# JaronTu/Multimodal_MVD_Seg

Measured on AMD Instinct MI355X. Metric: train-step samples/sec on 4-modality 128^3 patches (PlainConvUNet 3d_fullres, fp32), higher is better.
Workload: dtype f32; 1 GPU; BASELINE configs[1]: PlainConvUNet 3d_fullres 6 stages 31.2M params, 4x128x128x128 patch, 5 classes, fp32, DC+CE deep supervision, SGD-Nesterov+clip; per_gpu_batch=2, global_batch=2, parallelism=dp1, step_launch=one hipGraph replay per step (captured after 3 eager steps)

## Files before the change

### include/mvdseg_hip.h

```cpp
#ifndef MVDSEG_HIP_H
#define MVDSEG_HIP_H
#include <stddef.h>
#include <stdint.h>

#ifdef __cplusplus
extern "C" {
#endif

#define MVD_VERSION 100
#define MVD_MAX_TAPS 27

int mvd_version(void);
const char *mvd_last_error(void);
int mvd_has_mfma(void);
int mvd_set_conv_engine(int mode);
int mvd_set_wino_min_items(long n);

int mvd_pack_weight(const float *w, float *wf, float *wb, int K, int C, int T, int transposed, void *stream);

size_t mvd_conv_fwd_workspace_bytes(int N, long out_voxels, int K);
int mvd_conv3d_fwd(const float *x1, int C1, const float *x2, int C2, const float *wf, const float *bias, float *y,
                   int N, int D, int H, int W, int K, const int ksize[3], const int stride[3], void *ws,
                   size_t ws_bytes, void *stream);
int mvd_conv3d_dgrad(const float *dy, const float *wb, float *dx1, int C1, float *dx2, int C2, int N, int D, int H,
// ... 42 lines not shown
#define MVD_WG_MFMA 5
#define MVD_WG_WGRAD16 6
#define MVD_WG_WGRAD16Z 7
#define MVD_WG_WGRAD16ZS 8
#define MVD_WG_SCALAR 9
#define MVD_WG_PLAN_LEN 34
#define MVD_WGR_F4 1
#define MVD_WGR_F16 2
#define MVD_WGR_WINO 3
#define MVD_WGR_WINO2 4
#define MVD_WGR_WINO3 5
#define MVD_WGR_D 6
#define MVD_WGB_NONE 0
#define MVD_WGB_COLSUM 1
#define MVD_WGB_GENERIC 2
#define MVD_WGB_CONVT 3
#define MVD_WGB_SMALLC 4
#define MVD_WGB_WINO3 5
#define MVD_WGB_WINO2W12 6
#define MVD_WGB_SLOT28 7
#define MVD_WGB_ZMARCH 8
int mvd_conv_wgrad_plan(int transposed, int is_bf16, int N, int D, int H, int W, int C1, int C2, int K, const int ksize[3],
                        const int stride[3], size_t ws_bytes, int want_bias, int prologue, long *plan);
int mvd_conv_wgrad_last_kernel(void);
size_t mvd_conv3d_wgrad_workspace_bytes(int C, int K, int T, int N, int Do, int Ho, int Wo);
int mvd_conv3d_wgrad(const float *x1, int C1, const float *x2, int C2, const float *dy, float *dw, float *dbias,
                     int N, int D, int H, int W, int K, const int ksize[3], const int stride[3], void *ws,
                     size_t ws_bytes, void *stream);

int mvd_convT3d_fwd(const float *x, const float *wf, const float *bias, float *y, int N, int D, int H, int W, int C,
                    int K, const int stride[3], void *ws, size_t ws_bytes, void *stream);
int mvd_convT3d_dgrad(const float *dy, const float *wb, float *dx, int N, int D, int H, int W, int C, int K,
                      const int stride[3], void *ws, size_t ws_bytes, void *stream);
size_t mvd_convT3d_wgrad_workspace_bytes(int C, int K, int T, int N, int D, int H, int W);
int mvd_convT3d_wgrad(const float *x, const float *dy, float *dw, float *dbias, int N, int D, int H, int W, int C,
                      int K, const int stride[3], void *ws, size_t ws_bytes, void *stream);

int mvd_pack_weight_bf16(const float *w, uint16_t *wf, uint16_t *wb, int K, int C, int T, int transposed, void *stream);
int mvd_pack_weights_bf16_batch(int n, const float *const *w, uint16_t *const *wf, uint16_t *const *wb, const int *K,
                                const int *C, const int *T, const int *transposed, void *stream);
int mvd_pack_weights_bf16_batch_pad(int n, const float *const *w, uint16_t *const *wf, uint16_t *const *wb, const int *K,
                                    const int *C, const int *T, const int *transposed, const int *Csrc, void *stream);
int mvd_conv3d_fwd_bf16(const uint16_t *x1, int C1, const uint16_t *x2, int C2, const uint16_t *wf, const float *bias,
                        uint16_t *y, int N, int D, int H, int W, int K, const int ksize[3], const int stride[3],
                        void *ws, size_t ws_bytes, void *stream);
int mvd_conv3d_dgrad_bf16(const uint16_t *dy, const uint16_t *wb, uint16_t *dx1, int C1, uint16_t *dx2, int C2, int N,
                          int D, int H, int W, int K, const int ksize[3], const int stride[3], void *ws, size_t ws_bytes,
                          void *stream);
int mvd_convT3d_fwd_bf16(const uint16_t *x, const uint16_t *wf, const float *bias, uint16_t *y, int N, int D, int H, int W,
                         int C, int K, const int stride[3], void *ws, size_t ws_bytes, void *stream);
int mvd_convT3d_dgrad_bf16(const uint16_t *dy, const uint16_t *wb, uint16_t *dx, int N, int D, int H, int W, int C, int K,
                           const int stride[3], void *ws, size_t ws_bytes, void *stream);
int mvd_conv3d_wgrad_bf16(const uint16_t *x1, int C1, const uint16_t *x2, int C2, const uint16_t *dy, float *dw,
                          float *dbias, int N, int D, int H, int W, int K, const int ksize[3], const int stride[3],
                          void *ws, size_t ws_bytes, void *stream);
int mvd_convT3d_wgrad_bf16(const uint16_t *x, const uint16_t *dy, float *dw, float *dbias, int N, int D, int H, int W,
                           int C, int K, const int stride[3], void *ws, size_t ws_bytes, void *stream);
int mvd_conv3d_fwd_bf16_stats_tiles(int N, int D, int H, int W, int C1, int C2, int K, const int ksize[3],
                                    const int stride[3]);
int mvd_conv3d_dgrad_acc_ok(int is_bf16, int N, int D, int H, int W, int C1, int K, const int ksize[3], const int stride[3]);
int mvd_conv3d_dgrad_acc(const float *dy, const float *wb, float *dx1, int C1, int N, int D, int H, int W, int K,
                         const int ksize[3], const int stride[3], void *stream);
int mvd_conv3d_dgrad_bf16_acc(const uint16_t *dy, const uint16_t *wb, uint16_t *dx1, int C1, int N, int D, int H, int W, int K,
                              const int ksize[3], const int stride[3], void *ws, size_t ws_bytes, void *stream);
int mvd_set_bf16_zmarch_kernel(int which);
int mvd_set_bf16_wgrad_kernel(int which);
// ... 387 lines not shown
```

### multimodal_mvd_seg_amd/_lib.py

```python
import ctypes
import os
from ctypes import c_double, c_float, c_int, c_long, c_size_t, c_uint64, c_void_p

_HERE = os.path.dirname(os.path.abspath(__file__))
LIB_PATH = os.path.join(_HERE, "libmvdseg_hip.so")

_P = c_void_p
_I3 = ctypes.c_int * 3

CONV_DIRECT, CONV_WINO2, CONV_WINO3, CONV_WINO2P = 0, 1, 2, 3

SIGNATURES = {
    "mvd_version": (c_int, []),
    "mvd_last_error": (ctypes.c_char_p, []),
    "mvd_has_mfma": (c_int, []),
    "mvd_set_conv_engine": (c_int, [c_int]),
    "mvd_set_wino_min_items": (c_int, [c_long]),
    "mvd_pack_weight": (c_int, [_P, _P, _P, c_int, c_int, c_int, c_int, _P]),
    "mvd_conv_fwd_workspace_bytes": (c_size_t, [c_int, c_long, c_int]),
    "mvd_conv3d_fwd": (c_int, [_P, c_int, _P, c_int, _P, _P, _P, c_int, c_int, c_int, c_int, c_int, _I3, _I3, _P,
                               c_size_t, _P]),
    "mvd_conv3d_dgrad": (c_int, [_P, _P, _P, c_int, _P, c_int, c_int, c_int, c_int, c_int, c_int, _I3, _I3, _P,
                                 c_size_t, _P]),
    "mvd_conv3d_wgrad_workspace_bytes": (c_size_t, [c_int, c_int, c_int, c_int, c_int, c_int, c_int]),
    "mvd_conv3d_wgrad": (c_int, [_P, c_int, _P, c_int, _P, _P, _P, c_int, c_int, c_int, c_int, c_int, _I3, _I3, _P,
                                 c_size_t, _P]),
    "mvd_convT3d_fwd": (c_int, [_P, _P, _P, _P, c_int, c_int, c_int, c_int, c_int, c_int, _I3, _P, c_size_t, _P]),
    "mvd_convT3d_dgrad": (c_int, [_P, _P, _P, c_int, c_int, c_int, c_int, c_int, c_int, _I3, _P, c_size_t, _P]),
    "mvd_convT3d_wgrad_workspace_bytes": (c_size_t, [c_int, c_int, c_int, c_int, c_int, c_int, c_int]),
    "mvd_convT3d_wgrad": (c_int, [_P, _P, _P, _P, c_int, c_int, c_int, c_int, c_int, c_int, _I3, _P, c_size_t, _P]),
    "mvd_conv3d_route": (c_int, [c_int, c_int, c_int, c_int, c_int, c_int, c_int, _I3, _I3]),
    "mvd_conv3d_fwd_routed": (c_int, [_P, c_int, _P, c_int, _P, _P, c_int, _P, _P, _P, c_long, _P, c_int, c_int, c_int, c_int,
                                      c_int, _I3, _I3, _P, c_size_t, _P]),
    "mvd_conv3d_dgrad_routed": (c_int, [_P, _P, _P, c_int, _P, c_int, _P, c_int, c_int, c_int, c_int, c_int, c_int, _I3, _I3, _P,
                                        c_size_t, _P]),
    "mvd_conv_wino_applicable": (c_int, [c_int, c_int, c_int, c_int, c_int, c_int, c_int, _I3, _I3]),
    "mvd_wino_mode": (c_int, []),
    "mvd_wino_weight_elems": (c_size_t, [c_int, c_int]),
    "mvd_pack_weight_wino": (c_int, [_P, _P, _P, c_int, c_int, _P]),
    "mvd_conv3d_fwd_wino": (c_int, [_P, c_int, _P, c_int, _P, _P, _P, _P, c_int, c_int, c_int, c_int, c_int, _I3, _I3, _P,
                                    c_size_t, _P]),
    "mvd_conv_stats_tiles": (c_size_t, [c_int, c_int, c_int]),
    "mvd_conv3d_fwd_stats_tiles": (c_long, [c_int, c_int, c_int, c_int, c_int, c_int, c_int, _I3, _I3]),
    "mvd_set_wino3_min_items": (c_int, [c_long]),
    "mvd_conv_wino3_applicable": (c_int, [c_int, c_int, c_int, c_int, c_int, c_int, c_int, _I3, _I3]),
    "mvd_wino3_weight_elems": (c_size_t, [c_int, c_int]),
    "mvd_pack_weight_wino3": (c_int, [_P, _P, _P, c_int, c_int, _P]),
    "mvd_pack_weights_batch3": (c_int, [c_int] + [_P] * 11 + [_P]),
    "mvd_set_wino2p_min_items": (c_int, [c_long]),
    "mvd_conv_wino2p_applicable": (c_int, [c_int, c_int, c_int, c_int, c_int, c_int, c_int, _I3, _I3]),
    "mvd_wino2p_weight_elems": (c_size_t, [c_int, c_int]),
    "mvd_pack_weight_wino2p": (c_int, [_P, _P, _P, c_int, c_int, _P]),
    "mvd_set_wgrad_wino3_min_items": (c_int, [c_long]),
    "mvd_conv_wgrad_wino3_applicable": (c_int, [c_int, c_int, c_int, c_int, c_int, c_int, c_int, _I3, _I3]),
    "mvd_wgrad_wino3_launches": (c_long, []),
    "mvd_set_wgrad_bias_fold": (c_int, [c_int]),
    "mvd_conv_wgrad_plan": (c_int, [c_int, c_int, c_int, c_int, c_int, c_int, c_int, c_int, c_int, _I3, _I3, c_size_t, c_int,
                                    c_int, _P]),
    "mvd_conv_wgrad_last_kernel": (c_int, []),
    "mvd_conv3d_wgrad_bf16": (c_int, [_P, c_int, _P, c_int, _P, _P, _P, c_int, c_int, c_int, c_int, c_int, _I3, _I3, _P,
                                      c_size_t, _P]),
# ... 257 lines not shown
```

### multimodal_mvd_seg_amd/csrc/conv.hip

```cpp
#include "common.h"
#include "conv_geom.h"

namespace mvd {

static int g_engine_mode = 0;
#define g_wino_off (wino_mode() == 0)
static const int g_transp_off = getenv("MVD_TRANSP") ? (atoi(getenv("MVD_TRANSP")) == 0) : 0;
static long g_wino_min_items = getenv("MVD_WINO_MIN") ? atol(getenv("MVD_WINO_MIN")) : 256;
static const long kWino3MinItemsDefault = 128;
static long g_wino3_min_items = getenv("MVD_WINO3_MIN") ? atol(getenv("MVD_WINO3_MIN")) : kWino3MinItemsDefault;
static const long kWino2pMinItemsDefault = 256;
static long g_wino2p_min_items = getenv("MVD_WINO2P_MIN") ? atol(getenv("MVD_WINO2P_MIN")) : kWino2pMinItemsDefault;

struct ConvPass {
    int N, D, H, W, R1, R2, P1, P2;
    const int *ks, *st;
};
static ConvPass fwd_pass(int N, int D, int H, int W, int C1, int C2, int K, const int ks[3], const int st[3]) {
    return {N, D, H, W, C1, C2, K, 0, ks, st};
}
static ConvPass dgrad_pass(int N, int D, int H, int W, int C1, int C2, int K, const int ks[3], const int st[3]) {
    return {N, D, H, W, K, 0, C1, C2, ks, st};
}
static bool wino_pass_ok(const ConvPass &p, int kd) {
    if (g_engine_mode != 0 || g_wino_off || !p.ks || !p.st) return false;
    if (p.ks[0] != kd || p.ks[1] != 3 || p.ks[2] != 3 || p.st[0] != 1 || p.st[1] != 1 || p.st[2] != 1) return false;
    if (p.N <= 0 || p.D <= 0 || p.H <= 0 || p.W <= 0 || p.R1 <= 0 || p.R2 < 0 || p.P1 <= 0 || p.P2 < 0) return false;
    return !(p.R1 % 32 || p.R2 % 32 || p.P1 % 32 || p.P2 % 32);
}
static long wino2_items(int N, int D, int H, int W, int K) { return (long)N * ((D + 3) / 4) * ((H + 3) / 4) * ((W + 7) / 8) * (K / 32); }
static bool wino2_takes(const ConvPass &p) {
    return wino_pass_ok(p, 3) && wino2_items(p.N, p.D, p.H, p.W, p.P1 + p.P2) >= g_wino_min_items;
}
static long wino3_items(int D, int H, int W, int K) { return (long)((D + 3) / 4) * ((H + 7) / 8) * ((W + 7) / 8) * (K / 32); }
static bool wino3_takes(const ConvPass &p) {
    return wino3_enabled() && wino2_takes(p) && wino3_items(p.D, p.H, p.W, p.P1 + p.P2) >= g_wino3_min_items;
}
static bool wino2p_takes(const ConvPass &p) {
    if (!wino_pass_ok(p, 1)) return false;
    const int cmax = p.R1 + p.R2 > p.P1 + p.P2 ? p.R1 + p.R2 : p.P1 + p.P2;
// ... 582 lines not shown
    if (want_bias && !in_kernel_bias) p.bias_src = WGB_COLSUM;
    const long out[MVD_WG_PLAN_LEN] = {p.kernel, p.reduce, p.bias_src, p.TPW, p.NA, p.NB, p.SH, p.TRI, p.TD, p.TH, p.TW,
                                       p.ntd, p.nth, p.ntw, p.ntiles, p.nsplit, p.partials, p.ncb, p.nkb, p.bias_rows,
                                       (long)p.needed_ws, (long)p.ws_bytes, p.wino_mode, p.wino3_on, p.wino3_min_items,
                                       p.bias_fold, p.bf16_kernel, p.engine_mode, p.env_big16, p.env_tri16, p.env_db,
                                       p.env_16z, p.env_16zs, p.env_reduce_g16};
    for (int i = 0; i < MVD_WG_PLAN_LEN; i++) plan[i] = out[i];
    return 0;
}

int mvd_set_wgrad_bias_fold(int on) {
    set_wgrad_bias_fold(on);
    return 0;
}

int mvd_conv3d_wgrad(const float *x1, int C1, const float *x2, int C2, const float *dy, float *dw, float *dbias, int N,
                     int D, int H, int W, int K, const int ksize[3], const int stride[3], void *ws, size_t ws_bytes,
                     void *stream) {
    MVD_REQUIRE(x1 && dy && dw && ws && C1 > 0 && C2 >= 0 && (C2 == 0 || x2), "conv3d_wgrad: null pointer / bad channels");
    MVD_REQUIRE(N > 0 && D > 0 && H > 0 && W > 0 && K > 0, "conv3d_wgrad: bad shape");
    if (check_ks(ksize, stride, "conv3d_wgrad")) return 2;
    WgradGeom g;
    conv_wgrad_geom(g, N, D, H, W, C1, C2, K, ksize, stride);
    MVD_REQUIRE(ws_bytes >= mvd_conv3d_wgrad_workspace_bytes(C1 + C2, K, g.T, N, g.Do, g.Ho, g.Wo),
                "conv3d_wgrad: workspace too small");
    hipStream_t s = as_stream(stream);
    int dbias_done = 0;
    int r = run_wgrad(g, x1, x2, dy, dw, ws, ws_bytes, s, dbias, &dbias_done);
    if (r) return r;
    if (dbias && !dbias_done) return colsum(dy, dbias, (long)N * g.Do * g.Ho * g.Wo, K, ws, s);
    return 0;
}

int mvd_convT3d_fwd(const float *x, const float *wf, const float *bias, float *y, int N, int D, int H, int W, int C, int K,
                    const int stride[3], void *ws, size_t ws_bytes, void *stream) {
    MVD_REQUIRE(x && wf && y && N > 0 && D > 0 && H > 0 && W > 0 && C > 0 && K > 0, "convT3d_fwd: bad arguments");
    for (int a = 0; a < 3; a++) MVD_REQUIRE(stride[a] == 1 || stride[a] == 2, "convT3d_fwd: stride must be 1 or 2");
    if (g_engine_mode == 0 && !g_transp_off) {
        int r = convT_fwd_direct(x, wf, bias, y, N, D, H, W, C, K, stride, as_stream(stream));
        if (r >= 0) return r;
    }
    for (int pd = 0; pd < stride[0]; pd++)
        for (int ph = 0; ph < stride[1]; ph++)
            for (int pw = 0; pw < stride[2]; pw++) {
                const int p[3] = {pd, ph, pw};
                FwdGeom g;
                convT_fwd_class_geom(g, N, D, H, W, C, K, stride, p);
                int r = run_fwd(g, x, nullptr, wf, bias, y, nullptr, ws, ws_bytes, as_stream(stream));
                if (r) return r;
            }
    return 0;
}

int mvd_convT3d_dgrad(const float *dy, const float *wb, float *dx, int N, int D, int H, int W, int C, int K,
                      const int stride[3], void *ws, size_t ws_bytes, void *stream) {
    MVD_REQUIRE(dy && wb && dx && N > 0 && D > 0 && H > 0 && W > 0 && C > 0 && K > 0, "convT3d_dgrad: bad arguments");
    for (int a = 0; a < 3; a++) MVD_REQUIRE(stride[a] == 1 || stride[a] == 2, "convT3d_dgrad: stride must be 1 or 2");
    if (g_engine_mode == 0 && !g_transp_off) {
        int r = convT_dgrad_direct(dy, wb, dx, N, D, H, W, C, K, stride, as_stream(stream));
        if (r >= 0) return r;
    }
    FwdGeom g;
    convT_dgrad_geom(g, N, D, H, W, C, K, stride);
    return run_fwd(g, dy, nullptr, wb, nullptr, dx, nullptr, ws, ws_bytes, as_stream(stream));
}

size_t mvd_convT3d_wgrad_workspace_bytes(int C, int K, int T, int N, int D, int H, int W) {
    WgradGeom g;
    memset(&g, 0, sizeof(g));
    g.N = N; g.Do = D; g.Ho = H; g.Wo = W; g.C1 = C; g.K = K; g.ntaps = g.T = T;
    size_t a = max_sz(wgrad_scalar_ws(g), wgrad_mfma_ws(g));
    return max_sz(a, colsum_ws((long)N * D * H * W * T, K));
}

int mvd_convT3d_wgrad(const float *x, const float *dy, float *dw, float *dbias, int N, int D, int H, int W, int C, int K,
                      const int stride[3], void *ws, size_t ws_bytes, void *stream) {
    MVD_REQUIRE(x && dy && dw && ws && N > 0 && D > 0 && H > 0 && W > 0 && C > 0 && K > 0, "convT3d_wgrad: bad arguments");
    for (int a = 0; a < 3; a++) MVD_REQUIRE(stride[a] == 1 || stride[a] == 2, "convT3d_wgrad: stride must be 1 or 2");
    WgradGeom g;
    convT_wgrad_geom(g, N, D, H, W, C, K, stride);
    MVD_REQUIRE(ws_bytes >= mvd_convT3d_wgrad_workspace_bytes(C, K, g.T, N, D, H, W), "convT3d_wgrad: workspace too small");
    hipStream_t s = as_stream(stream);
    int dbias_done = 0;
    int r = run_wgrad(g, x, nullptr, dy, dw, ws, ws_bytes, s, dbias, &dbias_done);
    if (r) return r;
    if (dbias && !dbias_done) return colsum(dy, dbias, (long)N * g.Db * g.Hb * g.Wb, K, ws, s);
    return 0;
}

int mvd_pack_weight_bf16(const float *w, uint16_t *wf, uint16_t *wb, int K, int C, int T, int transposed, void *stream) {
    MVD_REQUIRE(w && (wf || wb) && K > 0 && C > 0 && T > 0 && T <= MVD_MAX_TAPS, "pack_weight_bf16: bad arguments");
    MVD_REQUIRE(!wf || C % 32 == 0, "pack_weight_bf16: wf needs C %% 32 == 0");
    MVD_REQUIRE(!wb || K % 32 == 0, "pack_weight_bf16: wb needs K %% 32 == 0");
    return pack_weight16(w, wf, wb, K, C, T, transposed, as_stream(stream));
// ... 257 lines not shown
```

### multimodal_mvd_seg_amd/csrc/conv_geom.h

```cpp
#pragma once
#include <hip/hip_runtime.h>
#include <stdint.h>
#include <string.h>

namespace mvd {

__host__ __device__ inline int wl_ck(int C) {
    return (C % 32 == 0) ? 32 : ((C % 8 == 0) ? 8 : ((C % 4 == 0) ? 4 : 0));
}
__host__ __device__ inline size_t widx(int CK, int T, int C, int K, int t, int c, int k) {
    if (CK == 0) return ((size_t)t * C + c) * K + k;
    const int hh = CK / 2;
    const int cc = c / CK, r = c % CK;
    return ((((size_t)cc * T + t) * 2 + r / hh) * K + k) * hh + (r % hh);
}

struct FwdGeom {
    int N;
    int T;
    int Di, Hi, Wi;
    int Do, Ho, Wo;
    int Dy, Hy, Wy;
    int C1, C2, K1, K2;
    int ntaps;
// ... 262 lines not shown

int fwd_wino(const FwdGeom &g, const float *a1, const float *a2, const float *u, const float *bias, float *y1, float *y2,
             hipStream_t s, float *stats = nullptr, int *stats_done = nullptr);
int pack_weight_wino(const float *w, float *uf, float *ub, int K, int C, hipStream_t s);
int fwd_wino3(const FwdGeom &g, const float *a1, const float *a2, const float *u, const float *bias, float *y1, float *y2,
              hipStream_t s, float *stats = nullptr, int *stats_done = nullptr);
int pack_weight_wino3(const float *w, float *uf, float *ub, int K, int C, hipStream_t s);
int wino3_enabled();
int fwd_wino2p(const FwdGeom &g, const float *a1, const float *a2, const float *u, const float *bias, float *y1, float *y2,
               hipStream_t s);
int pack_weight_wino2p(const float *w, float *uf, float *ub, int K, int C, hipStream_t s);
long wino2p_items(int N, int D, int H, int W, int K);
int dgrad32s(int N, int D, int H, int W, int C, int K, int Do, int Ho, int Wo, const float *dy, const float *wb, float *dx,
             hipStream_t s, int accumulate = 0);
int dgrad16s(int N, int D, int H, int W, int C, int K, int Do, int Ho, int Wo, const unsigned short *dy, const unsigned short *wb,
             unsigned short *dx, hipStream_t s, int accumulate = 0);
int launch_fwd16ys(const FwdGeom &g, const unsigned short *a1, const unsigned short *a2, const unsigned short *w, const float *bias,
                   unsigned short *y1, unsigned short *y2, hipStream_t s, int ncu);
bool wgrad16z_prologue_ok(const WgradGeom &g);
void wgrad16z_enable(int on);
int pack_weights_batch(int n, const float *const *w, float *const *wf, float *const *wb, float *const *uf, float *const *ub,
                       const int *K, const int *C, const int *T, const int *transposed, hipStream_t s,
                       float *const *vf = nullptr, float *const *vb = nullptr);
int wino_mode();
bool wgrad_wino3_selected(const WgradGeom &g);
size_t wgrad_wino3_ws(int nsplit, int C, int K);
int wgrad_wino3_enabled();
void set_wgrad_wino3_min_items(long n);
void set_wgrad_bias_fold(int on);
long wgrad_wino3_launches();
int dbias_reduce(const float *pbias, float *dbias, int K, int nrows, hipStream_t s);
size_t wino_weight_elems(int C, int K);

int convT_fwd_direct(const float *x, const float *wf, const float *bias, float *y, int N, int D, int H, int W, int C, int K,
                     const int st[3], hipStream_t s);
int convT_dgrad_direct(const float *dy, const float *wb, float *dx, int N, int D, int H, int W, int C, int K,
                       const int st[3], hipStream_t s);

int convT_fwd_direct16(const unsigned short *x, const unsigned short *wf, const float *bias, unsigned short *y, int N, int D,
                       int H, int W, int C, int K, const int st[3], hipStream_t s);
int convT_dgrad_direct16(const unsigned short *dy, const unsigned short *wb, unsigned short *dx, int N, int D, int H, int W,
                         int C, int K, const int st[3], hipStream_t s);

struct Fwd16Fuse {
    float *tile_stats = nullptr;
    int *ntiles = nullptr;
    const float *in_scale = nullptr, *in_shift = nullptr;
    float slope = 0.01f;
};
int fwd_bf16(const FwdGeom &g, const unsigned short *a1, const unsigned short *a2, const unsigned short *w,
             const float *bias, unsigned short *y1, unsigned short *y2, void *ws, size_t ws_bytes, hipStream_t s,
             const Fwd16Fuse *fuse = nullptr);
int fwd16y_enabled();
void fwd16y_enable(int on);
int launch_fwd16y(const FwdGeom &g, const unsigned short *a1, const unsigned short *a2, const unsigned short *w,
                  const float *bias, unsigned short *y1, unsigned short *y2, hipStream_t s, const Fwd16Fuse *fuse, int ncu,
                  int *stats_tiles_only);
int fwd_bf16_stats_tiles(const FwdGeom &g);
int fwd_bf16_prologue_ok(const FwdGeom &g);
int pack_weight16(const float *w, unsigned short *wf, unsigned short *wb, int K, int C, int T, int transposed,
                  hipStream_t s);
int pack_weights16_batch(int n, const float *const *w, unsigned short *const *wf, unsigned short *const *wb, const int *K,
                         const int *C, const int *T, const int *transposed, const int *Csrc, hipStream_t s);

}
```

### multimodal_mvd_seg_amd/csrc/conv_transp.hip

```cpp
#include <algorithm>
#include <stdlib.h>
#include "common.h"
#include "conv_geom.h"

namespace mvd {

typedef float f32x16 __attribute__((ext_vector_type(16)));

struct TranspGeom {
    int N, D, H, W, C, K;
    int s[3], T;
    long NV;
};

__device__ inline long out_base(const TranspGeom &g, unsigned v) {
    const unsigned t1 = v / (unsigned)g.W, w = v - t1 * (unsigned)g.W;
    const unsigned t2 = t1 / (unsigned)g.H, h = t1 - t2 * (unsigned)g.H;
    return (((long)t2 * g.s[0]) * (g.H * g.s[1]) + (long)h * g.s[1]) * (g.W * g.s[2]) + (long)w * g.s[2];
}

__global__ __launch_bounds__(256, 4) void k_convT_fwd(const TranspGeom g, const float *__restrict__ x,
                                                      const float *__restrict__ wf, const float *__restrict__ bias,
                                                      float *__restrict__ y) {
    const int lane = threadIdx.x & 63;
// ... 211 lines not shown
                for (int e = 0; e < 4; e++) a[u ^ 1][e] = *reinterpret_cast<const float4 *>(pa + e * 4);
#pragma unroll
                for (int q = 0; q < NT; q++)
#pragma unroll
                    for (int e = 0; e < 4; e++)
                        b[u ^ 1][q][e] = (cb0 + q < ncb) ? *reinterpret_cast<const float4 *>(pb + (size_t)q * 512 + e * 4)
                                                         : make_float4(0.f, 0.f, 0.f, 0.f);
#pragma unroll
                for (int e = 0; e < 4; e++) {
#pragma unroll
                    for (int q = 0; q < NT; q++) acc[q] = __builtin_amdgcn_mfma_f32_32x32x2f32(a[u][e].x, b[u][q][e].x, acc[q], 0, 0, 0);
#pragma unroll
                    for (int q = 0; q < NT; q++) acc[q] = __builtin_amdgcn_mfma_f32_32x32x2f32(a[u][e].y, b[u][q][e].y, acc[q], 0, 0, 0);
#pragma unroll
                    for (int q = 0; q < NT; q++) acc[q] = __builtin_amdgcn_mfma_f32_32x32x2f32(a[u][e].z, b[u][q][e].z, acc[q], 0, 0, 0);
#pragma unroll
                    for (int q = 0; q < NT; q++) acc[q] = __builtin_amdgcn_mfma_f32_32x32x2f32(a[u][e].w, b[u][q][e].w, acc[q], 0, 0, 0);
                }
            }
        }
    }
#pragma unroll
    for (int q = 0; q < NT; q++)
        if (cb0 + q < ncb) {
            const int c = (cb0 + q) * 32 + i;
#pragma unroll
            for (int r = 0; r < 16; r++) {
                const int row = (r & 3) + 8 * (r >> 2) + 4 * h;
                if (vb + row < g.NV) dx[(size_t)(vb + row) * g.C + c] = acc[q][r];
            }
        }
}

__global__ __launch_bounds__(256, 2) void k_convT_dgrad_p(const TranspGeom g, const float *__restrict__ dy,
                                                         const float *__restrict__ wb, float *__restrict__ dx, int ngrp) {
    const int lane = threadIdx.x & 63;
    const int wave = __builtin_amdgcn_readfirstlane(threadIdx.x >> 6);
    const int i = lane & 31, h = lane >> 5;
    const int ncb = g.C >> 5;
    const int cb = wave % ncb;
    const int gsub = wave / ncb, gper = 4 / ncb;
    const int Hy = g.H * g.s[1], Wy = g.W * g.s[2];
    const float *wl = wb + (((size_t)h * g.C + cb * 32 + i) << 4);
    const size_t wtap = (size_t)2 * g.C * 16;
    float4 wr[8][4];
    int poff[8];
#pragma unroll
    for (int p = 0; p < 8; p++) {
#pragma unroll
        for (int e = 0; e < 4; e++) wr[p][e] = *reinterpret_cast<const float4 *>(wl + (size_t)p * wtap + e * 4);
        const int pw = p % g.s[2], ph = (p / g.s[2]) % g.s[1], pd = p / (g.s[2] * g.s[1]);
        poff[p] = (pd * Hy + ph) * Wy + pw;
    }
    const int c = cb * 32 + i;
    const int gstride = (int)gridDim.x * gper;
    int grp = (int)blockIdx.x * gper + gsub;
    if (grp >= ngrp) return;
    auto row_ptr = [&](int gq) {
        const long vv = (long)gq * 32 + i;
        const long ob = out_base(g, (unsigned)(vv < g.NV ? vv : g.NV - 1));
        return dy + (size_t)ob * g.K + h * 16;
    };
    const float *rp = row_ptr(grp);
    float4 a[2][4];
#pragma unroll
    for (int e = 0; e < 4; e++) a[0][e] = *reinterpret_cast<const float4 *>(rp + (size_t)poff[0] * g.K + e * 4);
    for (; grp < ngrp; grp += gstride) {
        const int gn = grp + gstride < ngrp ? grp + gstride : grp;
        const float *rn = row_ptr(gn);
        f32x16 acc;
#pragma unroll
        for (int r = 0; r < 16; r++) acc[r] = 0.f;
#pragma unroll
        for (int p = 0; p < 8; p++) {
            const float *pn = p < 7 ? rp + (size_t)poff[p < 7 ? p + 1 : 0] * g.K : rn + (size_t)poff[0] * g.K;
#pragma unroll
            for (int e = 0; e < 4; e++) a[(p + 1) & 1][e] = *reinterpret_cast<const float4 *>(pn + e * 4);
#pragma unroll
            for (int e = 0; e < 4; e++) {
                acc = __builtin_amdgcn_mfma_f32_32x32x2f32(a[p & 1][e].x, wr[p][e].x, acc, 0, 0, 0);
                acc = __builtin_amdgcn_mfma_f32_32x32x2f32(a[p & 1][e].y, wr[p][e].y, acc, 0, 0, 0);
                acc = __builtin_amdgcn_mfma_f32_32x32x2f32(a[p & 1][e].z, wr[p][e].z, acc, 0, 0, 0);
                acc = __builtin_amdgcn_mfma_f32_32x32x2f32(a[p & 1][e].w, wr[p][e].w, acc, 0, 0, 0);
            }
        }
        const long vb = (long)grp * 32;
#pragma unroll
        for (int r = 0; r < 16; r++) {
            const int row = (r & 3) + 8 * (r >> 2) + 4 * h;
            if (vb + row < g.NV) dx[(size_t)(vb + row) * g.C + c] = acc[r];
        }
        rp = rn;
    }
}

typedef __bf16 bf16x8t __attribute__((ext_vector_type(8)));

__device__ inline bf16x8t ld_bf8(const unsigned short *p) {
    const uint4 q = *reinterpret_cast<const uint4 *>(p);
    return __builtin_bit_cast(bf16x8t, q);
}

__global__ __launch_bounds__(256, 4) void k_convT_fwd16(const TranspGeom g, const unsigned short *__restrict__ x,
                                                        const unsigned short *__restrict__ wf,
                                                        const float *__restrict__ bias, unsigned short *__restrict__ y) {
    const int lane = threadIdx.x & 63;
    const int wave = __builtin_amdgcn_readfirstlane(threadIdx.x >> 6);
    const int i = lane & 31, h = lane >> 5;
    const long vb = (long)blockIdx.x * 32;
    const int ppw = (g.T + 3) >> 2;
    const int p0 = wave * ppw;
    if (p0 >= g.T) return;
    const int kb = blockIdx.y;
    const int nch = g.C >> 5;
    const long v = vb + i < g.NV ? vb + i : g.NV - 1;
    const unsigned short *xl = x + (size_t)v * g.C + h * 8;
    const unsigned short *wl = wf + (((size_t)h * g.K + kb * 32 + i) << 3);
    const size_t ws_ = (size_t)2 * g.K * 8;
    const size_t wtap = 2 * ws_;
    f32x16 acc[2];
#pragma unroll
    for (int p = 0; p < 2; p++)
#pragma unroll
        for (int r = 0; r < 16; r++) acc[p][r] = 0.f;
    const int np = g.T - p0 < ppw ? g.T - p0 : ppw;
// ... 173 lines not shown
                load_ab(st + 1 < nsteps ? st + 1 : st, u ^ 1);
#pragma unroll
                for (int s2 = 0; s2 < 2; s2++)
#pragma unroll
                    for (int q = 0; q < NT; q++)
                        acc[q] = __builtin_amdgcn_mfma_f32_32x32x16_bf16(b[u][q][s2], a[u][s2], acc[q], 0, 0, 0);
            }
        }
    }
    if (vb + i < g.NV) {
#pragma unroll
        for (int q = 0; q < NT; q++)
            if (cb0 + q < ncb) {
                unsigned short *xo = dx + (size_t)v * g.C + (cb0 + q) * 32 + 4 * h;
#pragma unroll
                for (int rg = 0; rg < 4; rg++) {
                    uint2 pk;
                    pk.x = (unsigned)f2bf(acc[q][rg * 4 + 0]) | ((unsigned)f2bf(acc[q][rg * 4 + 1]) << 16);
                    pk.y = (unsigned)f2bf(acc[q][rg * 4 + 2]) | ((unsigned)f2bf(acc[q][rg * 4 + 3]) << 16);
                    *reinterpret_cast<uint2 *>(xo + 8 * rg) = pk;
                }
            }
    }
}

static bool transp_geom(TranspGeom &g, int N, int D, int H, int W, int C, int K, const int st[3]) {
    g.N = N; g.D = D; g.H = H; g.W = W; g.C = C; g.K = K;
    for (int a = 0; a < 3; a++) g.s[a] = st[a];
    g.T = st[0] * st[1] * st[2];
    g.NV = (long)N * D * H * W;
    return C % 32 == 0 && K % 32 == 0 && g.T <= 8 && g.NV * g.T < (1L << 31) && g.NV > 0;
}

int convT_fwd_direct(const float *x, const float *wf, const float *bias, float *y, int N, int D, int H, int W, int C, int K,
                     const int st[3], hipStream_t s) {
    TranspGeom g;
    if (!transp_geom(g, N, D, H, W, C, K, st)) return -1;
    if (((uintptr_t)x | (uintptr_t)wf) & 15) return -1;
    const long bx = (g.NV + 31) / 32;
    if (bx > (1L << 30) || K / 32 > 65535) return -1;
    static const int pers = getenv("MVD_CONVT_PERSIST") ? atoi(getenv("MVD_CONVT_PERSIST")) : 1;
    if (pers && g.T == 8 && C == 64 && K == 32 && bx >= 4096) {
        const unsigned gx = (unsigned)std::min<long>(bx, 512);
        hipLaunchKernelGGL(k_convT_fwd_p<2>, dim3(gx, 1), dim3(256), 0, s, g, x, wf, bias, y, (int)bx);
        return check_launch("convT fwd (persistent direct GEMM)");
    }
    hipLaunchKernelGGL(k_convT_fwd, dim3((unsigned)bx, K / 32), dim3(256), 0, s, g, x, wf, bias, y);
    return check_launch("convT fwd (direct GEMM)");
}

int convT_dgrad_direct(const float *dy, const float *wb, float *dx, int N, int D, int H, int W, int C, int K,
                       const int st[3], hipStream_t s) {
    TranspGeom g;
    if (!transp_geom(g, N, D, H, W, C, K, st)) return -1;
    if (((uintptr_t)dy | (uintptr_t)wb) & 15) return -1;
    const long bx = (g.NV + 127) / 128;
    if (bx > (1L << 30)) return -1;
    const int ncb = C / 32;
    static const int pers = getenv("MVD_CONVT_PERSIST") ? atoi(getenv("MVD_CONVT_PERSIST")) : 1;
    const long ngrp = (g.NV + 31) / 32;
    if (pers && g.T == 8 && K == 32 && (ncb == 1 || ncb == 2 || ncb == 4) && ngrp >= 4096 && ngrp < (1L << 30)) {
        const long nb = (ngrp * ncb + 3) / 4;
        hipLaunchKernelGGL(k_convT_dgrad_p, dim3((unsigned)std::min<long>(nb, 512)), dim3(256), 0, s, g, dy, wb, dx, (int)ngrp);
        return check_launch("convT dgrad (persistent direct GEMM)");
    }
    if (ncb > 4 && ncb % 2 == 0) {
        hipLaunchKernelGGL(k_convT_dgrad<2>, dim3((unsigned)bx, ncb / 2), dim3(256), 0, s, g, dy, wb, dx);
    } else {
        hipLaunchKernelGGL(k_convT_dgrad<1>, dim3((unsigned)bx, ncb), dim3(256), 0, s, g, dy, wb, dx);
    }
    return check_launch("convT dgrad (direct GEMM)");
}

int convT_fwd_direct16(const unsigned short *x, const unsigned short *wf, const float *bias, unsigned short *y, int N, int D,
                       int H, int W, int C, int K, const int st[3], hipStream_t s) {
    TranspGeom g;
    if (!transp_geom(g, N, D, H, W, C, K, st)) return -1;
    if (((uintptr_t)x | (uintptr_t)wf) & 15) return -1;
    const long bx = (g.NV + 31) / 32;
    if (bx > (1L << 30) || K / 32 > 65535) return -1;
    static const int pers = getenv("MVD_CONVT_PERSIST") ? atoi(getenv("MVD_CONVT_PERSIST")) : 1;
    if (pers && g.T == 8 && C == 64 && K == 32 && bx >= 4096) {
        hipLaunchKernelGGL(k_convT_fwd16_p, dim3((unsigned)std::min<long>(bx, 1024)), dim3(256), 0, s, g, x, wf, bias, y, (int)bx);
        return check_launch("convT fwd (bf16 persistent direct GEMM)");
    }
    hipLaunchKernelGGL(k_convT_fwd16, dim3((unsigned)bx, K / 32), dim3(256), 0, s, g, x, wf, bias, y);
    return check_launch("convT fwd (bf16 direct GEMM)");
}

int convT_dgrad_direct16(const unsigned short *dy, const unsigned short *wb, unsigned short *dx, int N, int D, int H, int W,
                         int C, int K, const int st[3], hipStream_t s) {
    TranspGeom g;
    if (!transp_geom(g, N, D, H, W, C, K, st)) return -1;
    if (((uintptr_t)dy | (uintptr_t)wb) & 15) return -1;
    const long bx = (g.NV + 127) / 128;
    if (bx > (1L << 30)) return -1;
    const int ncb = C / 32;
    if (ncb > 4 && ncb % 2 == 0)
        hipLaunchKernelGGL(k_convT_dgrad16<2>, dim3((unsigned)bx, ncb / 2), dim3(256), 0, s, g, dy, wb, dx);
    else
        hipLaunchKernelGGL(k_convT_dgrad16<1>, dim3((unsigned)bx, ncb), dim3(256), 0, s, g, dy, wb, dx);
    return check_launch("convT dgrad (bf16 direct GEMM)");
}

// ... 2 lines not shown
```

Baseline: 64.55 samples/s.

## Add split-reduce transposed-conv dgrad kernel and deeper prefetch ring

Adds a new transposed-conv dgrad kernel that splits the tap×K-chunk reduction across waves in a block and combines the partials through LDS, meant for small decoder levels where too few wavefronts would otherwise run. The same kernel in single-wave form uses a 4-deep register prefetch ring. The persistent dgrad kernel's ring depth becomes a template parameter and defaults to 4. A plan function chooses the kernel, and introspection and on/off entry points are exported. The costs are more register pressure from the deeper rings and extra LDS traffic and a block-wide sync for the reduction.

Result: no change. 65.00 samples/s, median of 6 (+0.7%).

```diff
diff --git a/include/mvdseg_hip.h b/include/mvdseg_hip.h
--- a/include/mvdseg_hip.h
+++ b/include/mvdseg_hip.h
@@ -98,6 +98,17 @@
                     int K, const int stride[3], void *ws, size_t ws_bytes, void *stream);
 int mvd_convT3d_dgrad(const float *dy, const float *wb, float *dx, int N, int D, int H, int W, int C, int K,
                       const int stride[3], void *ws, size_t ws_bytes, void *stream);
+#define MVD_CT_NONE 0
+#define MVD_CT_FWD 1
+#define MVD_CT_FWD_P 2
+#define MVD_CT_DGRAD1 3
+#define MVD_CT_DGRAD2 4
+#define MVD_CT_DGRAD_P 5
+#define MVD_CT_DGRAD_S 6
+#define MVD_CT_PLAN_LEN 10
+int mvd_convT_plan(int dgrad, int N, int D, int H, int W, int C, int K, const int stride[3], size_t ws_bytes, long *plan);
+int mvd_convT_last_kernel(void);
+int mvd_set_convT_direct(int on);
 size_t mvd_convT3d_wgrad_workspace_bytes(int C, int K, int T, int N, int D, int H, int W);
 int mvd_convT3d_wgrad(const float *x, const float *dy, float *dw, float *dbias, int N, int D, int H, int W, int C,
                       int K, const int stride[3], void *ws, size_t ws_bytes, void *stream);
diff --git a/multimodal_mvd_seg_amd/_lib.py b/multimodal_mvd_seg_amd/_lib.py
--- a/multimodal_mvd_seg_amd/_lib.py
+++ b/multimodal_mvd_seg_amd/_lib.py
@@ -27,6 +27,9 @@
                                  c_size_t, _P]),
     "mvd_convT3d_fwd": (c_int, [_P, _P, _P, _P, c_int, c_int, c_int, c_int, c_int, c_int, _I3, _P, c_size_t, _P]),
     "mvd_convT3d_dgrad": (c_int, [_P, _P, _P, c_int, c_int, c_int, c_int, c_int, c_int, _I3, _P, c_size_t, _P]),
+    "mvd_convT_plan": (c_int, [c_int, c_int, c_int, c_int, c_int, c_int, c_int, _I3, c_size_t, _P]),
+    "mvd_convT_last_kernel": (c_int, []),
+    "mvd_set_convT_direct": (c_int, [c_int]),
     "mvd_convT3d_wgrad_workspace_bytes": (c_size_t, [c_int, c_int, c_int, c_int, c_int, c_int, c_int]),
     "mvd_convT3d_wgrad": (c_int, [_P, _P, _P, _P, c_int, c_int, c_int, c_int, c_int, c_int, _I3, _P, c_size_t, _P]),
     "mvd_conv3d_route": (c_int, [c_int, c_int, c_int, c_int, c_int, c_int, c_int, _I3, _I3]),
diff --git a/multimodal_mvd_seg_amd/csrc/conv.hip b/multimodal_mvd_seg_amd/csrc/conv.hip
--- a/multimodal_mvd_seg_amd/csrc/conv.hip
+++ b/multimodal_mvd_seg_amd/csrc/conv.hip
@@ -5,7 +5,8 @@
 
 static int g_engine_mode = 0;
 #define g_wino_off (wino_mode() == 0)
-static const int g_transp_off = getenv("MVD_TRANSP") ? (atoi(getenv("MVD_TRANSP")) == 0) : 0;
+static int transp_off_env() { return getenv("MVD_TRANSP") ? (atoi(getenv("MVD_TRANSP")) == 0) : 0; }
+static int g_transp_off = transp_off_env();
 static long g_wino_min_items = getenv("MVD_WINO_MIN") ? atol(getenv("MVD_WINO_MIN")) : 256;
 static const long kWino3MinItemsDefault = 128;
 static long g_wino3_min_items = getenv("MVD_WINO3_MIN") ? atol(getenv("MVD_WINO3_MIN")) : kWino3MinItemsDefault;
@@ -654,6 +655,36 @@
     return 0;
 }
 
+static_assert(MVD_CT_NONE == CT_NONE && MVD_CT_FWD == CT_FWD && MVD_CT_FWD_P == CT_FWD_P && MVD_CT_DGRAD1 == CT_DGRAD1 && MVD_CT_DGRAD2 == CT_DGRAD2 && MVD_CT_DGRAD_P == CT_DGRAD_P &&
+                  MVD_CT_DGRAD_S == CT_DGRAD_S,
+              "transposed-conv kernel ids of the header and of conv_geom.h");
+
+int mvd_convT_last_kernel(void) { return g_convT_last_kernel; }
+
+int mvd_set_convT_direct(int on) {
+    g_transp_off = on < 0 ? transp_off_env() : on == 0;
+    return 0;
+}
+
+int mvd_convT_plan(int dgrad, int N, int D, int H, int W, int C, int K, const int stride[3], size_t ws_bytes, long *plan) {
+    MVD_REQUIRE(plan && stride && N > 0 && D > 0 && H > 0 && W > 0 && C > 0 && K > 0, "convT_plan: bad arguments");
+    for (int a = 0; a < 3; a++) MVD_REQUIRE(stride[a] == 1 || stride[a] == 2, "convT_plan: stride must be 1 or 2");
+    (void)ws_bytes;
+    ConvTPlan p;
+    const bool direct = convT_plan(dgrad != 0, N, D, H, W, C, K, stride, &p) && g_engine_mode == 0 && !g_transp_off;
+    if (!direct) {
+        p.kernel = CT_NONE;
+        p.split = 1;
+        p.depth = 0;
+        p.gx = p.gy = p.block = 0;
+        p.lds_bytes = 0;
+    }
+    const long out[MVD_CT_PLAN_LEN] = {p.kernel, p.split, p.depth, (long)p.gx, (long)p.gy, (long)p.block, (long)p.needed_ws,
+                                       (long)p.lds_bytes, p.env_persist, p.env_split};
+    for (int i = 0; i < MVD_CT_PLAN_LEN; i++) plan[i] = out[i];
+    return 0;
+}
+
 int mvd_convT3d_fwd(const float *x, const float *wf, const float *bias, float *y, int N, int D, int H, int W, int C, int K,
                     const int stride[3], void *ws, size_t ws_bytes, void *stream) {
     MVD_REQUIRE(x && wf && y && N > 0 && D > 0 && H > 0 && W > 0 && C > 0 && K > 0, "convT3d_fwd: bad arguments");
@@ -662,6 +693,7 @@
         int r = convT_fwd_direct(x, wf, bias, y, N, D, H, W, C, K, stride, as_stream(stream));
         if (r >= 0) return r;
     }
+    g_convT_last_kernel = CT_NONE;
     for (int pd = 0; pd < stride[0]; pd++)
         for (int ph = 0; ph < stride[1]; ph++)
             for (int pw = 0; pw < stride[2]; pw++) {
@@ -682,6 +714,7 @@
         int r = convT_dgrad_direct(dy, wb, dx, N, D, H, W, C, K, stride, as_stream(stream));
         if (r >= 0) return r;
     }
+    g_convT_last_kernel = CT_NONE;
     FwdGeom g;
     convT_dgrad_geom(g, N, D, H, W, C, K, stride);
     return run_fwd(g, dy, nullptr, wb, nullptr, dx, nullptr, ws, ws_bytes, as_stream(stream));
diff --git a/multimodal_mvd_seg_amd/csrc/conv_geom.h b/multimodal_mvd_seg_amd/csrc/conv_geom.h
--- a/multimodal_mvd_seg_amd/csrc/conv_geom.h
+++ b/multimodal_mvd_seg_amd/csrc/conv_geom.h
@@ -318,6 +318,19 @@
 int dbias_reduce(const float *pbias, float *dbias, int K, int nrows, hipStream_t s);
 size_t wino_weight_elems(int C, int K);
 
+enum { CT_NONE = 0, CT_FWD, CT_FWD_P, CT_DGRAD1, CT_DGRAD2, CT_DGRAD_P, CT_DGRAD_S };
+struct ConvTPlan {
+    int kernel;
+    int split;
+    int depth;
+    unsigned gx, gy, block;
+    size_t lds_bytes;
+    size_t needed_ws;
+    int env_persist, env_split;
+};
+bool convT_plan(bool dgrad, int N, int D, int H, int W, int C, int K, const int st[3], ConvTPlan *plan);
+extern int g_convT_last_kernel;
+
 int convT_fwd_direct(const float *x, const float *wf, const float *bias, float *y, int N, int D, int H, int W, int C, int K,
                      const int st[3], hipStream_t s);
 int convT_dgrad_direct(const float *dy, const float *wb, float *dx, int N, int D, int H, int W, int C, int K,
diff --git a/multimodal_mvd_seg_amd/csrc/conv_transp.hip b/multimodal_mvd_seg_amd/csrc/conv_transp.hip
--- a/multimodal_mvd_seg_amd/csrc/conv_transp.hip
+++ b/multimodal_mvd_seg_amd/csrc/conv_transp.hip
@@ -267,6 +267,7 @@
         }
 }
 
+template <int RING>
 __global__ __launch_bounds__(256, 2) void k_convT_dgrad_p(const TranspGeom g, const float *__restrict__ dy,
                                                          const float *__restrict__ wb, float *__restrict__ dx, int ngrp) {
     const int lane = threadIdx.x & 63;
@@ -297,9 +298,12 @@
         return dy + (size_t)ob * g.K + h * 16;
     };
     const float *rp = row_ptr(grp);
-    float4 a[2][4];
-#pragma unroll
-    for (int e = 0; e < 4; e++) a[0][e] = *reinterpret_cast<const float4 *>(rp + (size_t)poff[0] * g.K + e * 4);
+    static_assert(RING == 2 || RING == 4, "the ring divides the 8 positions");
+    float4 a[RING][4];
+#pragma unroll
+    for (int q = 0; q < RING - 1; q++)
+#pragma unroll
+        for (int e = 0; e < 4; e++) a[q][e] = *reinterpret_cast<const float4 *>(rp + (size_t)poff[q] * g.K + e * 4);
     for (; grp < ngrp; grp += gstride) {
         const int gn = grp + gstride < ngrp ? grp + gstride : grp;
         const float *rn = row_ptr(gn);
@@ -308,15 +312,16 @@
         for (int r = 0; r < 16; r++) acc[r] = 0.f;
 #pragma unroll
         for (int p = 0; p < 8; p++) {
-            const float *pn = p < 7 ? rp + (size_t)poff[p < 7 ? p + 1 : 0] * g.K : rn + (size_t)poff[0] * g.K;
-#pragma unroll
-            for (int e = 0; e < 4; e++) a[(p + 1) & 1][e] = *reinterpret_cast<const float4 *>(pn + e * 4);
+            const int q = p + RING - 1;
+            const float *pn = q < 8 ? rp + (size_t)poff[q & 7] * g.K : rn + (size_t)poff[q & 7] * g.K;
+#pragma unroll
+            for (int e = 0; e < 4; e++) a[q % RING][e] = *reinterpret_cast<const float4 *>(pn + e * 4);
 #pragma unroll
             for (int e = 0; e < 4; e++) {
-                acc = __builtin_amdgcn_mfma_f32_32x32x2f32(a[p & 1][e].x, wr[p][e].x, acc, 0, 0, 0);
-                acc = __builtin_amdgcn_mfma_f32_32x32x2f32(a[p & 1][e].y, wr[p][e].y, acc, 0, 0, 0);
-                acc = __builtin_amdgcn_mfma_f32_32x32x2f32(a[p & 1][e].z, wr[p][e].z, acc, 0, 0, 0);
-                acc = __builtin_amdgcn_mfma_f32_32x32x2f32(a[p & 1][e].w, wr[p][e].w, acc, 0, 0, 0);
+                acc = __builtin_amdgcn_mfma_f32_32x32x2f32(a[p % RING][e].x, wr[p][e].x, acc, 0, 0, 0);
+                acc = __builtin_amdgcn_mfma_f32_32x32x2f32(a[p % RING][e].y, wr[p][e].y, acc, 0, 0, 0);
+                acc = __builtin_amdgcn_mfma_f32_32x32x2f32(a[p % RING][e].z, wr[p][e].z, acc, 0, 0, 0);
+                acc = __builtin_amdgcn_mfma_f32_32x32x2f32(a[p % RING][e].w, wr[p][e].w, acc, 0, 0, 0);
             }
         }
         const long vb = (long)grp * 32;
@@ -326,6 +331,86 @@
             if (vb + row < g.NV) dx[(size_t)(vb + row) * g.C + c] = acc[r];
         }
         rp = rn;
+    }
+}
+
+__device__ __forceinline__ void mfma_step(f32x16 &acc, const float4 (&a)[4], const float4 (&b)[4]) {
+#pragma unroll
+    for (int e = 0; e < 4; e++) {
+        acc = __builtin_amdgcn_mfma_f32_32x32x2f32(a[e].x, b[e].x, acc, 0, 0, 0);
+        acc = __builtin_amdgcn_mfma_f32_32x32x2f32(a[e].y, b[e].y, acc, 0, 0, 0);
+        acc = __builtin_amdgcn_mfma_f32_32x32x2f32(a[e].z, b[e].z, acc, 0, 0, 0);
+        acc = __builtin_amdgcn_mfma_f32_32x32x2f32(a[e].w, b[e].w, acc, 0, 0, 0);
+    }
+}
+
+template <int NW>
+__global__ __launch_bounds__(NW == 1 ? 256 : 64 * NW) void k_convT_dgrad_s(const TranspGeom g, const float *__restrict__ dy,
+                                                                          const float *__restrict__ wb,
+                                                                          float *__restrict__ dx) {
+    __shared__ float red[NW == 1 ? 1 : NW * 16 * 64];
+    const int lane = threadIdx.x & 63;
+    const int wid = __builtin_amdgcn_readfirstlane(threadIdx.x >> 6);
+    const int wave = NW == 1 ? 0 : wid;
+    const int i = lane & 31, h = lane >> 5;
+    const long vb = NW == 1 ? ((long)blockIdx.x * 4 + wid) * 32 : (long)blockIdx.x * 32;
+    if (NW == 1 && vb >= g.NV) return;
+    const int cb = blockIdx.y;
+    const int nkc = g.K >> 5;
+    const int nsteps = g.T * nkc;
+    const int sb = nsteps * wave / NW, se = nsteps * (wave + 1) / NW;
+    const int sl = se - 1 > sb ? se - 1 : sb;
+    const long v = vb + i < g.NV ? vb + i : g.NV - 1;
+    const long ob = out_base(g, (unsigned)v);
+    const int Hy = g.H * g.s[1], Wy = g.W * g.s[2];
+    const float *wl = wb + (((size_t)h * g.C + cb * 32 + i) << 4);
+    const size_t wtap = (size_t)2 * g.C * 16;
+
+    f32x16 acc;
+#pragma unroll
+    for (int r = 0; r < 16; r++) acc[r] = 0.f;
+    float4 a[4][4], b[4][4];
+    auto load = [&](int step, float4 (&da)[4], float4 (&db)[4]) {
+        step = step < sl ? step : sl;
+        const int p = step / nkc, kc = step - p * nkc;
+        const int pw = p % g.s[2], ph = (p / g.s[2]) % g.s[1], pd = p / (g.s[2] * g.s[1]);
+        const float *pa = dy + (size_t)(ob + ((long)pd * Hy + ph) * Wy + pw) * g.K + kc * 32 + h * 16;
+        const float *pb = wl + ((size_t)kc * g.T + p) * wtap;
+#pragma unroll
+        for (int e = 0; e < 4; e++) da[e] = *reinterpret_cast<const float4 *>(pa + e * 4);
+#pragma unroll
+        for (int e = 0; e < 4; e++) db[e] = *reinterpret_cast<const float4 *>(pb + e * 4);
+    };
+    load(sb, a[0], b[0]);
+    load(sb + 1, a[1], b[1]);
+    load(sb + 2, a[2], b[2]);
+    for (int s0 = sb; s0 < se; s0 += 4) {
+#pragma unroll
+        for (int u = 0; u < 4; u++)
+            if (s0 + u < se) {
+                load(s0 + u + 3, a[(u + 3) & 3], b[(u + 3) & 3]);
+                mfma_step(acc, a[u], b[u]);
+            }
+    }
+    if (NW == 1) {
+#pragma unroll
+        for (int r = 0; r < 16; r++) {
+            const int row = (r & 3) + 8 * (r >> 2) + 4 * h;
+            if (vb + row < g.NV) dx[(size_t)(vb + row) * g.C + cb * 32 + i] = acc[r];
+        }
+        return;
+    }
+#pragma unroll
+    for (int r = 0; r < 16; r++) red[(wave * 16 + r) * 64 + lane] = acc[r];
+    __syncthreads();
+#pragma unroll
+    for (int j = 0; j < (NW > 1 ? 16 / NW : 0); j++) {
+        const int r = j * NW + wave;
+        float sum = red[r * 64 + lane];
+#pragma unroll
+        for (int w = 1; w < NW; w++) sum += red[(w * 16 + r) * 64 + lane];
+        const int row = (r & 3) + 8 * (r >> 2) + 4 * h;
+        if (vb + row < g.NV) dx[(size_t)(vb + row) * g.C + cb * 32 + i] = sum;
     }
 }
 
@@ -565,44 +650,119 @@
     return C % 32 == 0 && K % 32 == 0 && g.T <= 8 && g.NV * g.T < (1L << 31) && g.NV > 0;
 }
 
+static int convT_env(const char *name) {
+    const char *e = getenv(name);
+    return e ? atoi(e) : 1;
+}
+static const long kConvTFewWaves = 512;
+static const long kConvTFewWgs = 512;
+
+int g_convT_last_kernel = CT_NONE;
+
+bool convT_plan(bool dgrad, int N, int D, int H, int W, int C, int K, const int st[3], ConvTPlan *p) {
+    static const int pers = convT_env("MVD_CONVT_PERSIST"), split = convT_env("MVD_CONVT_SPLIT");
+    *p = ConvTPlan{};
+    p->kernel = CT_NONE;
+    p->split = 1;
+    p->depth = 2;
+    p->block = 256;
+    p->env_persist = pers;
+    p->env_split = split;
+    TranspGeom g;
+    if (!transp_geom(g, N, D, H, W, C, K, st)) return false;
+    const long ngrp = (g.NV + 31) / 32;
+    if (ngrp > (1L << 30) || K / 32 > 65535 || C / 32 > 65535) return false;
+    if (!dgrad) {
+        const int nkb = K / 32;
+        if (pers && g.T == 8 && C == 64 && K == 32 && ngrp >= 4096) {
+            p->kernel = CT_FWD_P;
+            p->gx = (unsigned)std::min<long>(ngrp, 512);
+            p->gy = 1;
+        } else {
+            p->kernel = CT_FWD;
+            p->gx = (unsigned)ngrp;
+            p->gy = (unsigned)nkb;
+        }
+        return true;
+    }
+    const int ncb = C / 32, nsteps = g.T * (K / 32);
+    if (pers && g.T == 8 && K == 32 && (ncb == 1 || ncb == 2 || ncb == 4) && ngrp >= 4096) {
+        const long nb = (ngrp * ncb + 3) / 4;
+        p->kernel = CT_DGRAD_P;
+        p->depth = split ? 4 : 2;
+        p->gx = (unsigned)std::min<long>(nb, 512);
+        p->gy = 1;
+        return true;
+    }
+    const int nt = ncb > 4 && ncb % 2 == 0 ? 2 : 1;
+    if (split && ngrp * (ncb / nt) <= kConvTFewWaves && nsteps >= 16) {
+        p->kernel = CT_DGRAD_S;
+        p->split = ngrp * ncb <= kConvTFewWgs && nsteps >= 32 ? 8 : 4;
+        p->depth = 4;
+        p->gx = (unsigned)ngrp;
+        p->gy = (unsigned)ncb;
+        p->block = 64u * p->split;
+        p->lds_bytes = (size_t)p->split * 16 * 64 * sizeof(float);
+        return true;
+    }
+    if (split && nt == 1 && nsteps >= 8) {
+        p->kernel = CT_DGRAD_S;
+        p->depth = 4;
+        p->gx = (unsigned)((g.NV + 127) / 128);
+        p->gy = (unsigned)ncb;
+        return true;
+    }
+    p->kernel = nt == 2 ? CT_DGRAD2 : CT_DGRAD1;
+    p->gx = (unsigned)((g.NV + 127) / 128);
+    p->gy = (unsigned)(ncb / nt);
+    return true;
+}
+
 int convT_fwd_direct(const float *x, const float *wf, const float *bias, float *y, int N, int D, int H, int W, int C, int K,
                      const int st[3], hipStream_t s) {
+    ConvTPlan p;
+    if (!convT_plan(false, N, D, H, W, C, K, st, &p)) return -1;
+    if (((uintptr_t)x | (uintptr_t)wf) & 15) return -1;
     TranspGeom g;
-    if (!transp_geom(g, N, D, H, W, C, K, st)) return -1;
-    if (((uintptr_t)x | (uintptr_t)wf) & 15) return -1;
-    const long bx = (g.NV + 31) / 32;
-    if (bx > (1L << 30) || K / 32 > 65535) return -1;
-    static const int pers = getenv("MVD_CONVT_PERSIST") ? atoi(getenv("MVD_CONVT_PERSIST")) : 1;
-    if (pers && g.T == 8 && C == 64 && K == 32 && bx >= 4096) {
-        const unsigned gx = (unsigned)std::min<long>(bx, 512);
-        hipLaunchKernelGGL(k_convT_fwd_p<2>, dim3(gx, 1), dim3(256), 0, s, g, x, wf, bias, y, (int)bx);
+    transp_geom(g, N, D, H, W, C, K, st);
+    const dim3 grid(p.gx, p.gy), block(p.block);
+    g_convT_last_kernel = p.kernel;
+    switch (p.kernel) {
+    case CT_FWD_P:
+        hipLaunchKernelGGL(k_convT_fwd_p<2>, grid, block, 0, s, g, x, wf, bias, y, (int)((g.NV + 31) / 32));
         return check_launch("convT fwd (persistent direct GEMM)");
-    }
-    hipLaunchKernelGGL(k_convT_fwd, dim3((unsigned)bx, K / 32), dim3(256), 0, s, g, x, wf, bias, y);
-    return check_launch("convT fwd (direct GEMM)");
+    default:
+        hipLaunchKernelGGL(k_convT_fwd, grid, block, 0, s, g, x, wf, bias, y);
+        return check_launch("convT fwd (direct GEMM)");
+    }
 }
 
 int convT_dgrad_direct(const float *dy, const float *wb, float *dx, int N, int D, int H, int W, int C, int K,
                        const int st[3], hipStream_t s) {
+    ConvTPlan p;
+    if (!convT_plan(true, N, D, H, W, C, K, st, &p)) return -1;
+    if (((uintptr_t)dy | (uintptr_t)wb) & 15) return -1;
     TranspGeom g;
-    if (!transp_geom(g, N, D, H, W, C, K, st)) return -1;
-    if (((uintptr_t)dy | (uintptr_t)wb) & 15) return -1;
-    const long bx = (g.NV + 127) / 128;
-    if (bx > (1L << 30)) return -1;
-    const int ncb = C / 32;
-    static const int pers = getenv("MVD_CONVT_PERSIST") ? atoi(getenv("MVD_CONVT_PERSIST")) : 1;
-    const long ngrp = (g.NV + 31) / 32;
-    if (pers && g.T == 8 && K == 32 && (ncb == 1 || ncb == 2 || ncb == 4) && ngrp >= 4096 && ngrp < (1L << 30)) {
-        const long nb = (ngrp * ncb + 3) / 4;
-        hipLaunchKernelGGL(k_convT_dgrad_p, dim3((unsigned)std::min<long>(nb, 512)), dim3(256), 0, s, g, dy, wb, dx, (int)ngrp);
+    transp_geom(g, N, D, H, W, C, K, st);
+    const dim3 grid(p.gx, p.gy), block(p.block);
+    g_convT_last_kernel = p.kernel;
+    switch (p.kernel) {
+    case CT_DGRAD_P:
+        if (p.depth == 4) hipLaunchKernelGGL(k_convT_dgrad_p<4>, grid, block, 0, s, g, dy, wb, dx, (int)((g.NV + 31) / 32));
+        else hipLaunchKernelGGL(k_convT_dgrad_p<2>, grid, block, 0, s, g, dy, wb, dx, (int)((g.NV + 31) / 32));
         return check_launch("convT dgrad (persistent direct GEMM)");
-    }
-    if (ncb > 4 && ncb % 2 == 0) {
-        hipLaunchKernelGGL(k_convT_dgrad<2>, dim3((unsigned)bx, ncb / 2), dim3(256), 0, s, g, dy, wb, dx);
-    } else {
-        hipLaunchKernelGGL(k_convT_dgrad<1>, dim3((unsigned)bx, ncb), dim3(256), 0, s, g, dy, wb, dx);
-    }
-    return check_launch("convT dgrad (direct GEMM)");
+    case CT_DGRAD_S:
+        if (p.split == 8) hipLaunchKernelGGL(k_convT_dgrad_s<8>, grid, block, 0, s, g, dy, wb, dx);
+        else if (p.split == 1) hipLaunchKernelGGL(k_convT_dgrad_s<1>, grid, block, 0, s, g, dy, wb, dx);
+        else hipLaunchKernelGGL(k_convT_dgrad_s<4>, grid, block, 0, s, g, dy, wb, dx);
+        return check_launch("convT dgrad (direct GEMM, split reduce)");
+    case CT_DGRAD2:
+        hipLaunchKernelGGL(k_convT_dgrad<2>, grid, block, 0, s, g, dy, wb, dx);
+        return check_launch("convT dgrad (direct GEMM)");
+    default:
+        hipLaunchKernelGGL(k_convT_dgrad<1>, grid, block, 0, s, g, dy, wb, dx);
+        return check_launch("convT dgrad (direct GEMM)");
+    }
 }
 
 int convT_fwd_direct16(const unsigned short *x, const unsigned short *wf, const float *bias, unsigned short *y, int N, int D,
```
